# biaslab/GaussianProcessNode

Hardware: AMD Instinct MI355X
Metric: VMP iterations/sec (sparse-GP node sweep, kin40k-shaped synthetic) (higher is better)
Workload: dtype f64

## Files before the change

### gaussianprocessnode_amd/csrc/sgp_api.hip

```cpp
#include "../../include/sgp_hip.h"
#include "sgp_kernels.hip.h"
#include "point_scratch.h"

#include <algorithm>
#include <atomic>
#include <chrono>
#include <cmath>
#include <cstdio>
#include <cstdlib>
#include <dlfcn.h>
#include <cstring>
#include <limits>
#include <mutex>
#include <string>
#include <type_traits>
#include <vector>

using namespace sgp;

namespace {

thread_local std::string g_create_error;
std::atomic<int> g_live_handles{0};

// ... 20 lines not shown
    std::lock_guard<std::mutex> lock(g_registry_mutex);
    auto& r = registry();
    auto it = std::find(r.begin(), r.end(), h);
    if (it == r.end()) return false;
    r.erase(it);
    return true;
}

}

enum { WORD_JOIN = 0,
       WORD_DONE = 1,
       WORD_GATE = 2,
       WORD_GRAD = 3,
       WORD_ASM0 = 4,
       WORD_GROUP0 = 8,
       WORD_COUNT = 8 + LAM_MAX_GROUPS };
constexpr int RESERVED_CUS_PER_SE = 2;

struct StatGroup {
    int c0, c1;
    int row_lo, nrows;
    int ntiles;
    SyrkGeom geom;
    int form_step;
    bool early;
    bool masked;
    size_t slab_off;
};

struct SweepPlan {
    hipStream_t stream = nullptr;
    bool overlapped = false;
    bool pack = false;
    bool events = false;
    bool join_word = false;
    bool kuu_interleaved = false;
    bool resident = false;
};

struct StatsRecord {
    double sigma2 = 0.0, jitter = 0.0, inv_ell[MAXD] = {0};
    int32_t family = SGP_KERNEL_SE;
    uint64_t data_gen = ~0ull;
    double w0 = 1.0;
    bool qv = false;
    bool reusable = false;
    bool checked = false;
    bool targets = false;
    bool exact_psi = false;
};
// ... 295 lines not shown
                               tv_xi, tv_t, mu_acc, uv_part, none);
        }
        ++j;
    }
};
static void launch_potrf(double* A, int ld, int Tn, int* info, int n_valid, double* scratch, hipStream_t s,
                         double* Winv = nullptr, const LamForm* form = nullptr, double* Sacc = nullptr,
                         const double* tv_xi = nullptr, double* tv_t = nullptr, const hipEvent_t* step_wait = nullptr) {
    PotrfSeq q(A, ld, Tn, info, n_valid, scratch, s, Winv, form, Sacc, tv_xi, tv_t, step_wait);
    while (!q.done()) q.next();
}

static void launch_ata(const double* W, double* C, int ld, int Tn, hipStream_t s, int rev = 0, double* mu = nullptr,
                       double* R = nullptr, const double* Psi2 = nullptr, const double* Kinv = nullptr,
                       double* trace_part = nullptr, const UvArgs* uv = nullptr, const double* Sacc = nullptr) {
    const int extra = uv ? Tn * Tn : 0;
    hipLaunchKernelGGL(k_gemm32, dim3(Tn * (Tn + 1) / 2 * 4 + extra), dim3(256), 0, s, W, W, C, ld, Tn, 0, 0, rev, mu, R, Psi2,
                       Kinv, trace_part, uv ? *uv : UvArgs{}, Sacc);
}
static void launch_gemm(const double* A, const double* B, double* C, int ld, int Tn, hipStream_t s) {
    hipLaunchKernelGGL(k_gemm32, dim3(Tn * Tn * 4), dim3(256), 0, s, A, B, C, ld, Tn, 3, 0, 0, (double*)nullptr, (double*)nullptr,
                       (const double*)nullptr, (const double*)nullptr, (double*)nullptr, UvArgs{}, (const double*)nullptr);
}


extern "C" int sgp_abi_version(void) { return SGP_ABI_VERSION; }

extern "C" const char* sgp_last_error(const sgp_handle* h) { return h ? h->err.c_str() : g_create_error.c_str(); }

template <typename T>
static hipError_t dalloc(T** p, size_t count) {
// ... 598 lines not shown
                           int64_t* stamps = nullptr, const long long* wait_word = nullptr, long long wait_need = 0,
                           const long long* gate_word = nullptr, long long gate_need = 0, int* sync_status = nullptr) {
    hipLaunchKernelGGL(k_prep_xu, dim3((h->Mp + 255) / 256), dim3(256), 0, s, h->dXu, Xus, src, dP, info_reset, h->M, h->Mp, h->D, stamps,
                       stamps ? (int)SGP_T_COUNT : 0, stamps ? (int)SGP_T_SWEEP : 0, wait_word, wait_need, gate_word, gate_need,
                       h->spin_limit, sync_status);
}
static void mirror_current_params(sgp_handle* h, hipStream_t s) { launch_prep_xu(h, s, h->dXusK, h->hParams, h->dParamsK); }

static void kuu_gram(sgp_handle* h, hipStream_t s, bool gate) {
    by_family(h->family, [&](auto F) {
        constexpr int FAM = decltype(F)::value;
        if (gate) hipLaunchKernelGGL(k_gram_uu_lds<FAM>, dim3(h->T, h->T), dim3(256), 0, s, h->dXusK, h->dKuu, h->dParamsK, h->M, h->Mp, h->D);
        else hipLaunchKernelGGL(k_gram_uu<FAM>, dim3(h->T, h->T), dim3(256), 0, s, h->dXusK, h->dKuu, h->dParamsK, h->M, h->Mp, h->D);
    });
}
static void kuu_tail(sgp_handle* h, hipStream_t s, bool join_word) {
    launch_ata(h->dWk, h->dKinv, h->Mp, h->T, s, 0, nullptr, nullptr, nullptr, nullptr, nullptr, nullptr, h->dSaccK);
    if (join_word) hipLaunchKernelGGL(k_join_set, dim3(1), dim3(64), 0, s, h->dJoin + WORD_JOIN, h->join_epoch);
}
static void enqueue_kuu_head(sgp_handle* h, hipStream_t s) {
    const bool words = s == h->side;
    const bool gate = words && h->gate_side;
    launch_prep_xu(h, s, h->dXusK, h->params_src, h->dParamsK, h->dInfo + 0, nullptr, words ? h->dJoin + WORD_DONE : nullptr,
                   h->done_epoch, gate ? h->dJoin + WORD_GATE : nullptr, h->gate_epoch, h->dInfo + 3);
    kuu_gram(h, s, gate);
}
static void enqueue_kuu(sgp_handle* h, hipStream_t s, bool join_word) {
    enqueue_kuu_head(h, s);
    launch_potrf(h->dKuu, h->Mp, h->T, h->dInfo + 0, h->M, h->dScratch, s, h->dWk, nullptr, h->dSaccK);
    kuu_tail(h, s, join_word);
}

static void launch_gram_uf(const sgp_handle* h, hipStream_t s, const double* Xus, const double* X, const double* Yw, double* Kuf,
                           double* bpart, const Params* P, int64_t N, int d_out, int64_t* stamps, int64_t* sweep_begin) {
    const dim3 grid((unsigned)((N + TB - 1) / TB), h->T);
    by_family(h->family, [&](auto F) {
        auto launch = [&](auto DCAP) {
            hipLaunchKernelGGL(HIP_KERNEL_NAME(k_gram_uf<decltype(DCAP)::value, decltype(F)::value>), grid, dim3(256), 0, s, Xus, X, Yw,
                               Kuf, bpart, P, h->M, h->Mp, h->D, N, d_out, stamps, sweep_begin);
        };
        if (h->D <= 8) launch(std::integral_constant<int, 8>{});
        else launch(std::integral_constant<int, MAXD>{});
    });
}
static void launch_gram(sgp_handle* h, hipStream_t s, bool stamped) {
// ... 51 lines not shown
            hipLaunchKernelGGL(k_join_set, dim3(1), dim3(64), 0, s, h->dJoin + WORD_GROUP0 + g, h->stat_epoch);
    }
    return 0;
}

static void enqueue_finish1(sgp_handle* h, hipStream_t s, const SweepPlan& p) {
    const int M = h->M, Mp = h->Mp, Q = h->Q, Qp = h->Qp, TQ = h->TQ;
    LamForm form;
    memset(&form, 0, sizeof form);
    form.stats = h->dStats; form.Lambda0 = h->dLambda0; form.xi0 = h->dXi0; form.xi = h->dXi; form.P = h->dParams;
    form.M = M; form.Mp = Mp; form.d_out = h->dout; form.Q = Q; form.prior_form = h->prior_form;
    form.stamps = h->dStamps + STAMP_STRIDE * SGP_T_FINISH1;
    form.spin_limit = h->spin_limit;
    form.sync_status = h->dInfo + 3;
    form.trace_chain = 1;
    hipEvent_t step_wait[LAM_MAX_COLS] = {nullptr};
    bool any_wait = false;
    if (p.overlapped) {
        form.col_words = h->dJoin + WORD_GROUP0;
        form.col_need = h->stat_epoch;
        for (int g = 0; g < h->ngroups; ++g) {
            for (int c = h->grp[g].c0; c < h->grp[g].c1; ++c) {
                form.form_step[c] = (unsigned char)(h->grp[g].form_step | (h->grp[g].early ? LAM_FORM_EARLY : 0));
                form.col_group[c] = (h->grp[g].masked && !p.pack && !p.resident) ? (unsigned char)g : (unsigned char)0xff;
            }
            if (h->grp[g].masked && p.pack && !p.resident) { step_wait[h->grp[g].form_step - (h->grp[g].early ? 1 : 0)] = h->evGroup[g]; any_wait = true; }
        }
    }
    double* uvt0 = h->dUvWork + 2 * (size_t)Qp;
    PotrfSeq lam(h->dLam, Qp, TQ, h->dInfo + 1, Qp, h->dScratch + POTRF_SCRATCH, s, h->dWl, &form, h->dTmp, h->dXi, uvt0,
                 any_wait ? step_wait : nullptr);
    lam.mu_acc = h->dUvWork;
    lam.uv_part = uvt0 + (size_t)TQ * Qp;
    if (p.kuu_interleaved) {
        PotrfSeq kuu(h->dKuu, h->Mp, h->T, h->dInfo + 0, h->M, h->dScratch, h->side, h->dWk, nullptr, h->dSaccK);
        while (!lam.done() || !kuu.done()) {
            if (!lam.done()) lam.next();
            if (!kuu.done()) kuu.next();
        }
        kuu_tail(h, h->side, p.join_word);
    } else {
        while (!lam.done()) lam.next();
    }
}

static double* mirror_for(const sgp_handle* h) {
    return (h->hMirror && !h->env_no_zero_copy && !h->training) ? h->hMirror : nullptr;
}

static void launch_traces(sgp_handle* h, hipStream_t s, const double* Rv = nullptr) {
    hipLaunchKernelGGL(k_trace_kinv, dim3(TRACE_BLOCKS), dim3(256), 0, s, h->dStats, h->dKinv, h->dTrace, h->M, h->Mp);
    hipLaunchKernelGGL(k_trace_R, dim3(TRACE_BLOCKS), dim3(256), 0, s, h->dStats, Rv ? Rv : h->dR, h->dTrace + TRACE_BLOCKS, h->M, h->Mp, h->dout,
                       h->Qp, (int64_t*)nullptr);
}

static void enqueue_finish2(sgp_handle* h, hipStream_t s, bool join_word) {
    const int M = h->M, Mp = h->Mp, Q = h->Q, Qp = h->Qp, TQ = h->TQ;
    double* uvt = h->dUvWork + 2 * (size_t)Qp;
    double* uvpart = uvt + (size_t)TQ * Qp;
    const int nata = TQ * (TQ + 1) / 2 * 4;
    double* traceR = h->dTrace + TRACE_BLOCKS;
    const double* partK = h->dTrace;
    int nK = TRACE_BLOCKS, nR = TRACE_BLOCKS;
    UvArgs uv;
    uv.Wp = h->dWl; uv.t = uvt; uv.muacc = h->dUvWork; uv.partial = uvpart; uv.LR = h->dUvT;
    uv.stamps = h->dStamps + STAMP_STRIDE * SGP_T_FINISH1;
    uv.join = join_word ? h->dJoin + WORD_JOIN : nullptr;
    uv.join_need = h->join_epoch;
    uv.spin_limit = h->spin_limit;
    uv.sync_status = h->dInfo + 3;
    if (h->dout == 1) {
        launch_ata(h->dWl, h->dSigma, Qp, TQ, s, 1, h->dMu, h->dR, h->dStats, h->dKinv, traceR, &uv, h->dTmp);
        partK = traceR + nata;
        nK = nR = nata;
    } else {
        launch_ata(h->dWl, h->dSigma, Qp, TQ, s, 1, h->dMu, h->dR, nullptr, nullptr, nullptr, &uv, h->dTmp);
        launch_traces(h, s);
    }
    hipLaunchKernelGGL(k_scalars, dim3(1), dim3(256), 0, s, h->dStats, partK, nK, (const double*)traceR, nR, h->dMu, h->dKuu,
                       h->dLam, h->dInfo, h->dParams, h->dOut, h->dWishart, M, Mp, h->dout, Q, Qp, Qp - Q,
                       h->dStamps + STAMP_STRIDE * SGP_T_FINISH2, h->dStamps, h->dStampTotals,
                       h->dJoin + WORD_DONE, h->done_epoch,
                       (const double*)(h->dScratch + POTRF_LOGDET), h->T, (const double*)(h->dScratch + POTRF_SCRATCH + POTRF_LOGDET), TQ,
                       mirror_for(h));
}

static int set_device_checked(int device) {
    int ndev = 0;
    if (hipGetDeviceCount(&ndev) != hipSuccess || ndev == 0) return fail(nullptr, SGP_ERR_NODEVICE, "no HIP device visible");
    if (device < 0 || device >= ndev) return fail(nullptr, SGP_ERR_ARG, "bad device ordinal");
    if (hipSetDevice(device) != hipSuccess) return fail(nullptr, SGP_ERR_HIP, "hipSetDevice failed");
    return 0;
}

namespace {
struct EventPair {
    hipEvent_t a = nullptr, b = nullptr;
    ~EventPair() { if (a) hipEventDestroy(a); if (b) hipEventDestroy(b); }
    hipError_t create() { hipError_t e = hipEventCreate(&a); return e != hipSuccess ? e : hipEventCreate(&b); }
// ... 39 lines not shown
    SweepPlan p;
    p.stream = stream ? static_cast<hipStream_t>(stream) : h->own;
    p.events = h->allreduce != nullptr || p.stream != h->own;
    p.overlapped = whole && h->overlap && !stream && (h->n > 0 || h->allreduce) && !h->training;
    p.pack = whole && h->allreduce != nullptr;
    return p;
}

static int sweep_local_impl(sgp_handle* h, void* stream, bool whole, bool need_data = true) {
    int rc = check_ready(h, need_data);
    if (rc) return rc;
    HIPCHK(h, hipSetDevice(h->cfg.device));
    SweepPlan p = sweep_plan(h, stream, whole);
    if (int brc = sweep_begin(h)) return brc;
    if (p.events) HIPCHK(h, hipStreamWaitEvent(h->side, h->evDone, 0));
    {
        const int grid = h->TQ * (h->TQ + 1) / 2 * 4 + h->TQ * h->TQ;
        p.join_word = h->dout == 1 && !p.events && grid <= h->num_cus - 40 && g_live_handles.load() <= 1;
        ++h->join_epoch;
    }
    ++h->gate_epoch;
    if (p.overlapped) ++h->stat_epoch;
    const bool stats_first = h->gate_side && h->n > 0 && !h->allreduce;
    p.kuu_interleaved = whole && h->env_interleave && stats_first && !p.events;
    h->plan = p;
    auto enqueue_stats = [&]() -> int {
        if (p.overlapped) {
            if (int orc = enqueue_stats_overlapped(h, p)) return orc;
        } else
            enqueue_local(h, p.stream, p.pack);
        HIPCHK(h, hipGetLastError());
        return 0;
    };
    if (stats_first)
        if (int src = enqueue_stats()) return src;
    if (p.kuu_interleaved)
        enqueue_kuu_head(h, h->side);
    else
        enqueue_kuu(h, h->side, p.join_word);
    HIPCHK(h, hipGetLastError());
    if (!p.kuu_interleaved) HIPCHK(h, hipEventRecord(h->evSide, h->side));
    if (!stats_first)
        if (int src = enqueue_stats()) return src;
    stats_formed(h);
    return 0;
}

extern "C" int sgp_sweep_local(sgp_handle* h, void* stream) {
    const int rc = sweep_local_impl(h, stream, false);
    if (h) stats_drop(h, STATS_REUSE);
    return rc;
}

extern "C" int sgp_sweep_finish(sgp_handle* h, void* stream) {
    if (!h) return SGP_ERR_ARG;
    if (!h->swept_local) return fail(h, SGP_ERR_ARG, "sgp_sweep_finish: call sgp_sweep_local first");
    HIPCHK(h, hipSetDevice(h->cfg.device));
    hipStream_t s = stream ? static_cast<hipStream_t>(stream) : h->own;
    const SweepPlan p = h->plan;
    h->plan.overlapped = h->plan.kuu_interleaved = false;
    h->in_flight = true;
    enqueue_finish1(h, s, p);
    HIPCHK(h, hipGetLastError());
    if (p.kuu_interleaved) HIPCHK(h, hipEventRecord(h->evSide, h->side));
    if (!p.join_word) HIPCHK(h, hipStreamWaitEvent(s, h->evSide, 0));
    return sweep_close(h, s, p, p.join_word);
}

static int exchange_stats(sgp_handle* h, hipStream_t s, int tile0, int ntile, bool with_tail) {
    const int tail = (int)(h->Mp * h->dout + SGP_S_COUNT + h->dout * h->dout);
    const int64_t count = (int64_t)ntile * TB * TB + (with_tail ? tail : 0);
    if (with_tail && tile0 + ntile != h->ntiles) return fail(h, SGP_ERR_ARG, "internal: the tail of the exchange buffer follows its last tile");
    if (h->allreduce(h->allreduce_ctx, h->dPack + (size_t)tile0 * TB * TB, count, s))
        return fail(h, SGP_ERR_HIP, "the all-reduce hook failed (statistics)");
    hipLaunchKernelGGL(k_unpack_stats, dim3(ntile + 1), dim3(256), 0, s, (const double*)h->dPack, h->dStats, h->Mp, h->T,
                       with_tail ? tail : 0, tile0, ntile);
    HIPCHK(h, hipGetLastError());
    return 0;
}
// ... 186 lines not shown

static bool mirror_fresh(const sgp_handle* h) {
    return h->hMirror && h->mirror_epoch >= 0 && h->mirror_epoch == h->done_epoch && !h->sync_reported &&
           h->hMirror[SGP_R_COUNT + 1] == (double)h->mirror_epoch;
}

static int check_sync_status(sgp_handle* h) {
    if (mirror_fresh(h) && h->hMirror[SGP_R_COUNT] == 0.0) return 0;
    int bits = 0;
    HIPCHK(h, hipMemcpy(&bits, h->dInfo + 3, sizeof(int), hipMemcpyDeviceToHost));
    if (bits == 0) return 0;
    h->sync_reported = true;
    std::string msg = "a bounded device-word wait gave up (stream hand-off not honoured; results refused):";
    if (bits & SYNC_LATE_DONE) msg += " [done word: the next sweep's first kernels started before the previous sweep had finished]";
    if (bits & SYNC_LATE_GRAD_START) msg += " [done word: the K_uu half of the theta gradient started before the sweep had finished]";
    if (bits & SYNC_LATE_KINV) msg += " [join word: the Sigma launch did not get K_uu^-1 from the K_uu chain]";
    if (bits & SYNC_LATE_GRAD_JOIN) msg += " [gradient word: the K_uu half of the theta gradient did not arrive]";
    if (bits & SYNC_LATE_COLUMN) msg += " [statistics words: a Lambda-chain step did not get its tile columns / the masked stream did not get K_uf]";
    h->err = msg;
    return SGP_ERR_HIP;
}

static int sync_checked(sgp_handle* h) {
    if (int rc = sync_all(h)) return rc;
    return check_sync_status(h);
}

static int last_sweep_status(sgp_handle* h, const char* name_kuu, const char* name_lambda) {
    if (int src = check_sync_status(h)) return src;
    int info[2];
    HIPCHK(h, hipMemcpy(info, h->dInfo, sizeof info, hipMemcpyDeviceToHost));
    return factor_status(h, info[0], name_kuu, info[1], name_lambda, true);
}
// ... 904 lines not shown
        if (int rrc = theta_Rv(h, s, &R)) return rrc;
    const int64_t nprep = std::max<int64_t>(h->n, Mp);
    hipLaunchKernelGGL(k_theta_multi_prep, dim3((unsigned)((nprep + 255) / 256)), dim3(256), 0, s, (const double*)h->dYw,
                       (const double*)h->dMu, w.W, cw, mup, h->n, M, Mp, dout);
    hipLaunchKernelGGL(k_form_G_multi, dim3(Mp), dim3(256), 0, s, R, Qp, (const double*)h->dKinv, (const double*)h->dStats,
                       w.W, w.trace, h->dGradM, part, M, Mp, dout);
    hipLaunchKernelGGL(k_theta_value_multi, dim3(1), dim3(256), 0, s, (const double*)part, (const double*)h->dStats,
                       (const double*)mup, (const Params*)h->dParams, w.W, w.trace, h->dGrad + GRAD_SLOTS, Mp, dout);
    HIPCHK(h, hipGetLastError());
    return 0;
}

static int enqueue_restats(sgp_handle* h, hipStream_t s) {
    stats_drop(h, STATS_REUSE | STATS_QV);
    h->swept_local = true;
    enqueue_kuu(h, s, false);
    enqueue_local(h, s, h->allreduce != nullptr);
    if (h->allreduce)
        if (int xrc = exchange_stats(h, s)) return xrc;
    force_prep_main(h);
    return 0;
}

static int theta_objective_multi(sgp_handle* h, hipStream_t s, bool fresh, double* value, double* grad) {
    if (fresh) {
        double out[SGP_R_COUNT];
        HIPCHK(h, hipMemcpy(out, h->dOut, sizeof out, hipMemcpyDeviceToHost));
        if (int frc = factor_status(h, (int)out[SGP_R_INFO_KUU], "K_uu")) return frc;
    } else {
        if (int erc = enqueue_restats(h, s)) return erc;
        HIPCHK(h, hipStreamSynchronize(s));
// ... 9 lines not shown
    HIPCHK(h, hipGetLastError());
    double res[GRAD_SLOTS + 1];
    HIPCHK(h, hipMemcpy(res, h->dGrad, sizeof res, hipMemcpyDeviceToHost));
    *value = res[GRAD_SLOTS];
    if (grad)
        for (int i = 0; i <= h->n_ell; ++i) grad[i] = res[i];
    return 0;
}

static void enqueue_theta_uni_sums(sgp_handle* h, hipStream_t s, const double* Rv) {
    const int M = h->M, Mp = h->Mp, Q = h->Q, Qp = h->Qp;
    launch_traces(h, s, Rv);
    hipLaunchKernelGGL(k_scalars, dim3(1), dim3(256), 0, s, h->dStats, (const double*)h->dTrace, (int)TRACE_BLOCKS,
                       (const double*)(h->dTrace + TRACE_BLOCKS), (int)TRACE_BLOCKS, h->dMu, h->dKuu, h->dLam, h->dInfo, h->dParams,
                       h->dOut2, h->dWishart, M, Mp, h->dout, Q, Qp, Qp - Q, (int64_t*)nullptr, (int64_t*)nullptr,
                       (int64_t*)nullptr, (long long*)nullptr, 0LL, (const double*)nullptr, 0, (const double*)nullptr, 0, (double*)nullptr);
}

static int theta_objective_eval(sgp_handle* h, hipStream_t s, double* value, const double** Rv_out) {
    if (int erc = enqueue_restats(h, s)) return erc;
    const int Mp = h->Mp;
    const double* Rv = h->dR;
    if (int rrc = theta_Rv(h, s, &Rv)) return rrc;
    *Rv_out = Rv;
    enqueue_theta_uni_sums(h, s, Rv);
    HIPCHK(h, hipStreamSynchronize(s));
    HIPCHK(h, hipGetLastError());
    double out[SGP_R_COUNT], sc[SGP_S_COUNT];
    HIPCHK(h, hipMemcpy(out, h->dOut2, sizeof out, hipMemcpyDeviceToHost));
    HIPCHK(h, hipMemcpy(sc, h->dStats + (size_t)Mp * Mp + (size_t)Mp * h->dout, sizeof sc, hipMemcpyDeviceToHost));
    if (int frc = factor_status(h, (int)out[SGP_R_INFO_KUU], "K_uu")) return frc;
// ... 841 lines not shown
```

### gaussianprocessnode_amd/csrc/sgp_kernels.hip.h

```cpp
#pragma once
#include <hip/hip_runtime.h>
#include <stdint.h>
#include <utility>

namespace sgp {

constexpr int TB = 64;
constexpr int PS = 80;
constexpr int KB = 16;
constexpr int MAXD = 32;
constexpr int MAXO = 4;
constexpr int LT = TB + 1;

typedef double d4 __attribute__((ext_vector_type(4)));

struct Params {
    double sigma2;
    double jitter;
    double E_logw;
    double n_override;
    double inv_ell[MAXD];
    double W[MAXO * MAXO];
    double prior_iso;
    double pad[7];
// ... 1213 lines not shown
constexpr int LAM_FORM_EARLY = 0x80;
struct LamForm {
    const double* stats;
    const double* Lambda0;
    const double* xi0;
    double* xi;
    const Params* P;
    int M, Mp, d_out, Q, prior_form;
    int64_t* stamps;
    const long long* col_words;
    long long col_need;
    unsigned char form_step[LAM_MAX_COLS], col_group[LAM_MAX_COLS];
    int spin_limit;
    int* sync_status;
    int trace_chain;
};
__device__ __forceinline__ double load_agent(const double* p) {
    return __hip_atomic_load((const __attribute__((address_space(1))) double*)p, __ATOMIC_RELAXED, __HIP_MEMORY_SCOPE_AGENT);
}
template <bool DENSE, bool MULTI, bool BYPASS = false>
__device__ __forceinline__ double lambda_entry(const LamForm& f, int gi, int gj, int Qp, double prior_iso, double w00) {
    const bool inside = gi < f.Q && gj < f.Q;
    const int si = inside ? gi : 0, sj = inside ? gj : 0;
    int a = 0, i = si, b = 0, j = sj;
    if constexpr (MULTI) { a = si / f.M; i = si % f.M; b = sj / f.M; j = sj % f.M; }
    double psi;
    if constexpr (BYPASS) psi = load_agent(f.stats + (size_t)j * f.Mp + i); else psi = f.stats[(size_t)j * f.Mp + i];
    const double diag = (gi == gj) ? 1.0 : 0.0;
    double prior, w;
    if constexpr (DENSE) prior = f.Lambda0[(size_t)sj * Qp + si]; else prior = diag * prior_iso;
// ... 496 lines not shown
    };
    TileRegs rX, rS, rD;
    if (lam && j == 0) stamp_enter(form.stamps);
    STEP_TRACE(0);
    if (panel) {
        long long* tw_words = reinterpret_cast<long long*>(scratch + 3 * TB * TB);
        if (!xgroup) {
            if (a != 0 || diag_inv) __builtin_amdgcn_s_setprio(3);
            tile_fetch(rS, do_form, load_old, A, form, ld, j0, j0, bypass);
            if (j > 0) {
                tile_g2r(rD, Dn_in, TB, 0, 0);
#pragma unroll
                for (int u = 0; u < 16; ++u) rS.v[u] -= rD.v[u];
            }
            if (xi_duty) form_xi(form, ld, tid, bypass);
            if (a == 0 && tid == 0) tw_words[(j + 1) & 1] = 0;
            tile_r2s(S, rS);
            STEP_TRACE(1);
            __syncthreads();
            STEP_TRACE(2);
            if (a == 0 && j > 0 && !diag_inv) move_prev();
            const bool has_solve = (a != 0) || diag_inv;
            const int ntwf = 1 + potrf_twins(Tn, j);
            static_assert(10 <= 2 * 2 * (1 + POTRF_TWINS), "two tiles of X X^T per wave must cover the ten lower tiles");
            int fcount = 0, fR[2], fC[2];
            d4 fg[2];
#pragma unroll
            for (int q = 0; q < 2; ++q) {
                fg[q] = (d4){0.0, 0.0, 0.0, 0.0};
                fR[q] = fC[q] = 0;
                const int t = tw + ntwf * ((wave - 1) + 2 * q);
// ... 159 lines not shown
#pragma unroll
    for (int u = 0; u < 32; ++u) {
        const double2 w = src[u];
        v[63 - 2 * u] = w.x;
        v[62 - 2 * u] = w.y;
    }
}

struct UvArgs {
    const double* Wp;
    const double* t;
    const double* muacc;
    const double* partial;
    double* LR;
    int64_t* stamps;
    const long long* join;
    long long join_need;
    int spin_limit;
    int* sync_status;
};
__global__ void k_join_wait(const long long* w, long long need, int spin_limit, int* sync_status, int bit, int trace_slot) {
    TraceScope trace(trace_slot);
    if (threadIdx.x == 0 && blockIdx.x == 0) spin_until(w, need, spin_limit, sync_status, bit);
}
__global__ void k_join_set(long long* w, long long v) {
    if (threadIdx.x == 0 && blockIdx.x == 0)
        __hip_atomic_store((__attribute__((address_space(1))) long long*)w, v, __ATOMIC_RELAXED, __HIP_MEMORY_SCOPE_AGENT);
}
__device__ __forceinline__ void uv_cols_role(const UvArgs& u, int Qp, int kb, int jb) {
    const int lane = threadIdx.x, j = 64 * jb + lane;
    double* out = u.LR + (size_t)(64 * kb) * Qp + j;
    if (kb > jb) {
#pragma unroll 16
        for (int kk = 0; kk < 64; ++kk) out[(size_t)kk * Qp] = 0.0;
        stamp_exit(u.stamps);
        return;
    }
    double v[64];
    load_v_column(v, u.Wp, Qp, kb, j);
    double T = 0.0;
// ... 35 lines not shown
        T = fma(lane_value(pl, kk), v[kk], T);
    }
    stamp_exit(u.stamps);
}

__global__ void __launch_bounds__(256) k_gemm32(const double* __restrict__ A, const double* __restrict__ B, double* __restrict__ C,
                                                int ld, int Tn, int mode, int s, int rev, double* __restrict__ mu,
                                                double* __restrict__ R, const double* __restrict__ Psi2,
                                                const double* __restrict__ Kinv, double* __restrict__ trace_part, UvArgs uv,
                                                const double* __restrict__ Sacc) {
    __shared__ double As[64 * PS32];
    __shared__ double Bs[64 * PS32];
    __shared__ double tred[4];
    __shared__ double mup[4 * 64], mus[64];
    TraceScope trace(mode == 0 ? (mu ? 5 : 6) : 255);
    if (mode == 0 && uv.Wp) {
        const int ngemm = Tn * (Tn + 1) / 2 * 4;
        if ((int)blockIdx.x >= ngemm) {
            if (threadIdx.x >= 64) return;
            const int e = blockIdx.x - ngemm;
            uv_cols_role(uv, ld, e % Tn, e / Tn);
            return;
        }
    }
    const int tid = threadIdx.x, lane = tid & 63, wave = tid >> 6, wr = wave >> 1, wc = wave & 1;
    const int quad = blockIdx.x & 3, qi = quad >> 1, qj = quad & 1;
    int I, J, kbeg, kend;
    if (mode == 0) {
        tile_from_index(blockIdx.x >> 2, I, J);
        kbeg = Sacc ? max(I, Tn - 2) : I;
        kend = Tn;
    } else {
        const int t = blockIdx.x >> 2;
        I = t / Tn; J = t % Tn; kbeg = 0; kend = Tn;
    }
    const int r0 = I * TB + qi * 32, c0 = J * TB + qj * 32;
    d4 acc = (d4){0.0, 0.0, 0.0, 0.0};
    const int li = lane & 15, lk = lane >> 4;
    if (mode == 0 && Sacc && I < Tn - 2) {
#pragma unroll
        for (int r = 0; r < 4; ++r) acc[r] = Sacc[(size_t)(c0 + wc * 16 + li) * ld + r0 + wr * 16 + lk + 4 * r];
    }
    const int oc = tid >> 3, o4 = (tid & 7) * 4;
    const int gcA = rev ? ld - 1 - (c0 + oc) : c0 + oc, grA = rev ? ld - 1 - (r0 + o4 + 3) : r0 + o4;
    const int gcB = rev ? ld - 1 - (r0 + oc) : r0 + oc, grB = rev ? ld - 1 - (c0 + o4 + 3) : c0 + o4;
    const size_t offA = (size_t)gcA * ld + grA, offB = (size_t)gcB * ld + grB;
    double2 p0 = make_double2(0.0, 0.0), p1 = p0, q0 = p0, q1 = p0;
    double muA[5] = {0.0, 0.0, 0.0, 0.0, 0.0}, muB[5] = {0.0, 0.0, 0.0, 0.0, 0.0};
    const int me = tid & 63;
    double mt[16], mbase = 0.0;
    bool kinv_late = false;
    if (mode == 0 && mu) {
#pragma unroll
        for (int u = 0; u < 16; ++u) mt[u] = uv.t[(Tn - 1) * TB + 16 * wave + u];
        if (wave == 0 && ((me < 32) ? I : J) < Tn - 1) mbase = uv.muacc[(me < 32) ? r0 + me : c0 + me - 32];
        if (Psi2) {
            p0 = *reinterpret_cast<const double2*>(Psi2 + offA); p1 = *reinterpret_cast<const double2*>(Psi2 + offA + 2);
            kinv_late = uv.join && !join_ready(uv.join, uv.join_need);
            if (!kinv_late) { q0 = *reinterpret_cast<const double2*>(Kinv + offA); q1 = *reinterpret_cast<const double2*>(Kinv + offA + 2); }
        }
    }
    for (int k = kbeg; k < kend; ++k) {
        __syncthreads();
        if (mode == 0) load_panel32_t(As, A, ld, k * TB, r0, tid);
        else load_panel32_n(As, A, ld, r0, k * TB, tid);
        load_panel32_t(Bs, B, ld, k * TB, c0, tid);
        __syncthreads();
        const double* ap = As + lk * PS32 + wr * 16 + li;
        const double* bp = Bs + lk * PS32 + wc * 16 + li;
#pragma unroll
        for (int k4 = 0; k4 < 16; ++k4) acc = __builtin_amdgcn_mfma_f64_16x16x4f64(ap[k4 * 4 * PS32], bp[k4 * 4 * PS32], acc, 0, 0, 0);
    }
    if (mode == 0 && mu) {
        const double* pan = ((me < 32) ? As + me : Bs + me - 32) + 16 * wave * PS32;
        double sdot = 0.0;
// ... 26 lines not shown
    }
    {
        double v[4];
#pragma unroll
        for (int e = 0; e < 4; ++e) v[e] = Qd[oc * 33 + o4 + (rev ? 3 - e : e)];
        *reinterpret_cast<double2*>(C + offA) = make_double2(v[0], v[1]);
        *reinterpret_cast<double2*>(C + offA + 2) = make_double2(v[2], v[3]);
        if (mu) {
            double rv[4];
#pragma unroll
            for (int e = 0; e < 4; ++e) rv[e] = fma(muA[e], muA[4], v[e]);
            *reinterpret_cast<double2*>(R + offA) = make_double2(rv[0], rv[1]);
            *reinterpret_cast<double2*>(R + offA + 2) = make_double2(rv[2], rv[3]);
            if (Psi2) {
                tsum = fma(rv[0], p0.x, fma(rv[1], p0.y, fma(rv[2], p1.x, rv[3] * p1.y)));
                if (kinv_late) {
                    if (spin_until(uv.join, uv.join_need, uv.spin_limit, uv.sync_status, SYNC_LATE_KINV)) {
                        const __attribute__((address_space(1))) double* kq = (const __attribute__((address_space(1))) double*)(Kinv + offA);
                        q0.x = __hip_atomic_load(kq + 0, __ATOMIC_RELAXED, __HIP_MEMORY_SCOPE_AGENT);
                        q0.y = __hip_atomic_load(kq + 1, __ATOMIC_RELAXED, __HIP_MEMORY_SCOPE_AGENT);
                        q1.x = __hip_atomic_load(kq + 2, __ATOMIC_RELAXED, __HIP_MEMORY_SCOPE_AGENT);
                        q1.y = __hip_atomic_load(kq + 3, __ATOMIC_RELAXED, __HIP_MEMORY_SCOPE_AGENT);
                    } else
                        q0.x = __builtin_nan("");
                }
                tsumK = fma(q0.x, p0.x, fma(q0.y, p0.y, fma(q1.x, p1.x, q1.y * p1.y)));
            }
        }
    }
    {
        double v[4];
#pragma unroll
        for (int e = 0; e < 4; ++e) v[e] = Qd[(o4 + (rev ? 3 - e : e)) * 33 + oc];
        *reinterpret_cast<double2*>(C + offB) = make_double2(v[0], v[1]);
        *reinterpret_cast<double2*>(C + offB + 2) = make_double2(v[2], v[3]);
        if (mu) {
            double rv[4];
#pragma unroll
            for (int e = 0; e < 4; ++e) rv[e] = fma(muB[e], muB[4], v[e]);
            *reinterpret_cast<double2*>(R + offB) = make_double2(rv[0], rv[1]);
            *reinterpret_cast<double2*>(R + offB + 2) = make_double2(rv[2], rv[3]);
        }
    }
    if (trace_part) {
        if (I != J) { tsum *= 2.0; tsumK *= 2.0; }
        tsum = block_sum(tsum, tred);
        tsumK = block_sum(tsumK, tred);
        if (tid == 0) {
            trace_part[blockIdx.x] = tsum;
            trace_part[Tn * (Tn + 1) / 2 * 4 + blockIdx.x] = tsumK;
        }
    }
}

__global__ void __launch_bounds__(256) k_symv(const double* __restrict__ S, const double* __restrict__ x,
                                              double* __restrict__ y, int n, int ld) {
    const int row = blockIdx.x * 4 + (threadIdx.x >> 6), lane = threadIdx.x & 63;
    if (row >= n) return;
    double s = 0.0;
    for (int j = lane; j < n; j += 64) s = fma(S[(size_t)row * ld + j], x[j], s);
    for (int o = 32; o > 0; o >>= 1) s += __shfl_xor(s, o);
    if (lane == 0) y[row] = s;
}

constexpr int CU_MAXQ = 4096;
// ... 29 lines not shown
                    t2 = fma(R[(size_t)(b * M + j) * Qp + a * M + i], Psi2[(size_t)j * Mp + i], t2);
            t2 = block_sum(t2, red);
            if (tid == 0) partial[(size_t)blockIdx.x * d_out * d_out + a + b * d_out] = t2;
        }
}

__global__ void __launch_bounds__(256) k_scalars(const double* __restrict__ stats, const double* __restrict__ partK, int nK,
                                                 const double* __restrict__ partR, int nR,
                                                 const double* __restrict__ mu, const double* __restrict__ Lkuu,
                                                 const double* __restrict__ Llam, const int* __restrict__ info,
                                                 const Params* __restrict__ P, double* __restrict__ out,
                                                 double* __restrict__ wishart, int M, int Mp, int d_out, int Q, int Qp,
                                                 int lam_off, int64_t* stamps, int64_t* all_stamps,
                                                 int64_t* totals, long long* done_word, long long done_value,
                                                 const double* __restrict__ ldK, int nldK, const double* __restrict__ ldL, int nldL,
                                                 double* __restrict__ mirror) {
    __shared__ double red[4];
    __shared__ double redn[4 * 5];
    __shared__ double tr[TRACE_SLOTS];
    TraceScope trace(7);
    stamp_enter(stamps);
    const double* B = stats + (size_t)Mp * Mp;
    const double* sc = B + (size_t)Mp * d_out;
    const int tid = threadIdx.x;
    if (d_out == 1) {
        StampFold fold = {0, 0, 0};
        if (all_stamps && tid >= 192) fold = stamp_fold_load(all_stamps, totals, tid - 192);
        const double c_syy = sc[0], c_skk = sc[1], c_n = sc[2], c_w = P->W[0], c_sigma2 = P->sigma2, c_elogw = P->E_logw;
        const int c_i0 = info[0], c_i1 = info[1], c_i2 = info[2], c_i3 = mirror ? info[3] : 0;
        double v[5] = {0.0, 0.0, 0.0, 0.0, 0.0};
        for (int b = tid; b < nK; b += 256) v[0] += partK[b];
        for (int b = tid; b < nR; b += 256) v[1] += partR[b];
        for (int e = tid; e < M; e += 256) {
            if (!ldK) v[2] += log(Lkuu[(size_t)e * Mp + e]);
            v[4] = fma(B[e], mu[e], v[4]);
        }
        if (ldK) for (int e = tid; e < nldK; e += 256) v[2] += ldK[e];
        if (ldL) for (int e = tid; e < nldL; e += 256) v[3] += ldL[e];
        else for (int e = tid; e < Q; e += 256) v[3] += log(Llam[(size_t)(e + lam_off) * Qp + e + lam_off]);
#pragma unroll
        for (int i = 0; i < 5; ++i)
            for (int o = 32; o > 0; o >>= 1) v[i] += __shfl_xor(v[i], o);
        if ((tid & 63) == 0)
#pragma unroll
            for (int i = 0; i < 5; ++i) redn[(tid >> 6) * 5 + i] = v[i];
        __syncthreads();
        if (tid == 0) {
            double t[5];
#pragma unroll
            for (int i = 0; i < 5; ++i) t[i] = (redn[i] + redn[5 + i]) + (redn[10 + i] + redn[15 + i]);
            const double LOG2PI = 1.8378770664093454835606594728112;
            const double n = c_n, w = c_w;
            const double sum_I1 = c_sigma2 * c_skk - t[0];
            const double sum_I2 = c_syy - 2.0 * t[4] + t[1];
// ... 2336 lines not shown
```

Before: 4835.

## Move K_uu trace term into Kinv launch and defer join to scalars kernel

The K_uu^-1 tail launch now also computes the trace(Kinv·Psi2) partials itself. It spin-waits on a new stats word that the Lambda-chain's first step publishes, plus any masked group words. The Sigma launch no longer waits on the join word for Kinv; only the closing scalars kernel spins on it to collect the traces and log-determinant. When the plan is not interleaved, the tail launch is deferred to the finish phase. The join-word path is also no longer gated by a CU-count budget, which takes the K_uu chain off the Sigma launch's critical path. The cost is extra device-word spinning and a risk of co-residency deadlock on the spin waits.

Result: no change. 4840, median of 6 (+0.1%).

```diff
diff --git a/gaussianprocessnode_amd/csrc/sgp_api.hip b/gaussianprocessnode_amd/csrc/sgp_api.hip
--- a/gaussianprocessnode_amd/csrc/sgp_api.hip
+++ b/gaussianprocessnode_amd/csrc/sgp_api.hip
@@ -58,6 +58,7 @@
        WORD_GATE = 2,
        WORD_GRAD = 3,
        WORD_ASM0 = 4,
+       WORD_STATS0 = 5,
        WORD_GROUP0 = 8,
        WORD_COUNT = 8 + LAM_MAX_GROUPS };
 constexpr int RESERVED_CUS_PER_SE = 2;
@@ -79,6 +80,7 @@
     bool pack = false;
     bool events = false;
     bool join_word = false;
+    bool kuu_tail_pending = false;
     bool kuu_interleaved = false;
     bool resident = false;
 };
@@ -404,7 +406,7 @@
 static void launch_ata(const double* W, double* C, int ld, int Tn, hipStream_t s, int rev = 0, double* mu = nullptr,
                        double* R = nullptr, const double* Psi2 = nullptr, const double* Kinv = nullptr,
                        double* trace_part = nullptr, const UvArgs* uv = nullptr, const double* Sacc = nullptr) {
-    const int extra = uv ? Tn * Tn : 0;
+    const int extra = (uv && uv->Wp) ? Tn * Tn : 0;
     hipLaunchKernelGGL(k_gemm32, dim3(Tn * (Tn + 1) / 2 * 4 + extra), dim3(256), 0, s, W, W, C, ld, Tn, 0, 0, rev, mu, R, Psi2,
                        Kinv, trace_part, uv ? *uv : UvArgs{}, Sacc);
 }
@@ -1033,9 +1035,23 @@
         else hipLaunchKernelGGL(k_gram_uu<FAM>, dim3(h->T, h->T), dim3(256), 0, s, h->dXusK, h->dKuu, h->dParamsK, h->M, h->Mp, h->D);
     });
 }
-static void kuu_tail(sgp_handle* h, hipStream_t s, bool join_word) {
-    launch_ata(h->dWk, h->dKinv, h->Mp, h->T, s, 0, nullptr, nullptr, nullptr, nullptr, nullptr, nullptr, h->dSaccK);
-    if (join_word) hipLaunchKernelGGL(k_join_set, dim3(1), dim3(64), 0, s, h->dJoin + WORD_JOIN, h->join_epoch);
+static double* kshares_of(const sgp_handle* h) { return h->dTrace + TRACE_BLOCKS + h->TQ * (h->TQ + 1) / 2 * 4; }
+static void kuu_tail(sgp_handle* h, hipStream_t s, const SweepPlan& p) {
+    if (p.join_word) {
+        UvArgs uv{};
+        uv.stat_word = h->dJoin + WORD_STATS0;
+        uv.stat_need = h->join_epoch;
+        uv.group_words = h->dJoin + WORD_GROUP0;
+        uv.group_need = h->stat_epoch;
+        if (p.overlapped && !p.pack)
+            for (int g = 0; g < h->ngroups; ++g)
+                if (h->grp[g].masked) uv.group_mask |= 1u << g;
+        uv.spin_limit = h->spin_limit;
+        uv.sync_status = h->dInfo + 3;
+        launch_ata(h->dWk, h->dKinv, h->Mp, h->T, s, 0, nullptr, nullptr, h->dStats, nullptr, kshares_of(h), &uv, h->dSaccK);
+        hipLaunchKernelGGL(k_join_set, dim3(1), dim3(64), 0, s, h->dJoin + WORD_JOIN, h->join_epoch, 11);
+    } else
+        launch_ata(h->dWk, h->dKinv, h->Mp, h->T, s, 0, nullptr, nullptr, nullptr, nullptr, nullptr, nullptr, h->dSaccK);
 }
 static void enqueue_kuu_head(sgp_handle* h, hipStream_t s) {
     const bool words = s == h->side;
@@ -1044,10 +1060,10 @@
                    h->done_epoch, gate ? h->dJoin + WORD_GATE : nullptr, h->gate_epoch, h->dInfo + 3);
     kuu_gram(h, s, gate);
 }
-static void enqueue_kuu(sgp_handle* h, hipStream_t s, bool join_word) {
+static void enqueue_kuu(sgp_handle* h, hipStream_t s, const SweepPlan& p, bool tail) {
     enqueue_kuu_head(h, s);
     launch_potrf(h->dKuu, h->Mp, h->T, h->dInfo + 0, h->M, h->dScratch, s, h->dWk, nullptr, h->dSaccK);
-    kuu_tail(h, s, join_word);
+    if (tail) kuu_tail(h, s, p);
 }
 
 static void launch_gram_uf(const sgp_handle* h, hipStream_t s, const double* Xus, const double* X, const double* Yw, double* Kuf,
@@ -1129,6 +1145,7 @@
     form.spin_limit = h->spin_limit;
     form.sync_status = h->dInfo + 3;
     form.trace_chain = 1;
+    if (p.join_word) { form.stats0_word = h->dJoin + WORD_STATS0; form.stats0_value = h->join_epoch; }
     hipEvent_t step_wait[LAM_MAX_COLS] = {nullptr};
     bool any_wait = false;
     if (p.overlapped) {
@@ -1153,7 +1170,7 @@
             if (!lam.done()) lam.next();
             if (!kuu.done()) kuu.next();
         }
-        kuu_tail(h, h->side, p.join_word);
+        kuu_tail(h, h->side, p);
     } else {
         while (!lam.done()) lam.next();
     }
@@ -1180,12 +1197,13 @@
     UvArgs uv;
     uv.Wp = h->dWl; uv.t = uvt; uv.muacc = h->dUvWork; uv.partial = uvpart; uv.LR = h->dUvT;
     uv.stamps = h->dStamps + STAMP_STRIDE * SGP_T_FINISH1;
-    uv.join = join_word ? h->dJoin + WORD_JOIN : nullptr;
-    uv.join_need = h->join_epoch;
+    uv.stat_word = uv.group_words = nullptr;
+    uv.stat_need = uv.group_need = 0;
+    uv.group_mask = 0;
     uv.spin_limit = h->spin_limit;
     uv.sync_status = h->dInfo + 3;
     if (h->dout == 1) {
-        launch_ata(h->dWl, h->dSigma, Qp, TQ, s, 1, h->dMu, h->dR, h->dStats, h->dKinv, traceR, &uv, h->dTmp);
+        launch_ata(h->dWl, h->dSigma, Qp, TQ, s, 1, h->dMu, h->dR, h->dStats, join_word ? nullptr : h->dKinv, traceR, &uv, h->dTmp);
         partK = traceR + nata;
         nK = nR = nata;
     } else {
@@ -1197,7 +1215,8 @@
                        h->dStamps + STAMP_STRIDE * SGP_T_FINISH2, h->dStamps, h->dStampTotals,
                        h->dJoin + WORD_DONE, h->done_epoch,
                        (const double*)(h->dScratch + POTRF_LOGDET), h->T, (const double*)(h->dScratch + POTRF_SCRATCH + POTRF_LOGDET), TQ,
-                       mirror_for(h));
+                       mirror_for(h), join_word ? (const long long*)(h->dJoin + WORD_JOIN) : (const long long*)nullptr, h->join_epoch,
+                       h->spin_limit, h->dInfo + 3);
 }
 
 static int set_device_checked(int device) {
@@ -1267,15 +1286,13 @@
     SweepPlan p = sweep_plan(h, stream, whole);
     if (int brc = sweep_begin(h)) return brc;
     if (p.events) HIPCHK(h, hipStreamWaitEvent(h->side, h->evDone, 0));
-    {
-        const int grid = h->TQ * (h->TQ + 1) / 2 * 4 + h->TQ * h->TQ;
-        p.join_word = h->dout == 1 && !p.events && grid <= h->num_cus - 40 && g_live_handles.load() <= 1;
-        ++h->join_epoch;
-    }
+    p.join_word = h->dout == 1 && !p.events && g_live_handles.load() <= 1;
+    ++h->join_epoch;
     ++h->gate_epoch;
     if (p.overlapped) ++h->stat_epoch;
     const bool stats_first = h->gate_side && h->n > 0 && !h->allreduce;
     p.kuu_interleaved = whole && h->env_interleave && stats_first && !p.events;
+    p.kuu_tail_pending = p.join_word && !p.kuu_interleaved;
     h->plan = p;
     auto enqueue_stats = [&]() -> int {
         if (p.overlapped) {
@@ -1290,7 +1307,7 @@
     if (p.kuu_interleaved)
         enqueue_kuu_head(h, h->side);
     else
-        enqueue_kuu(h, h->side, p.join_word);
+        enqueue_kuu(h, h->side, p, !p.kuu_tail_pending);
     HIPCHK(h, hipGetLastError());
     if (!p.kuu_interleaved) HIPCHK(h, hipEventRecord(h->evSide, h->side));
     if (!stats_first)
@@ -1311,11 +1328,12 @@
     HIPCHK(h, hipSetDevice(h->cfg.device));
     hipStream_t s = stream ? static_cast<hipStream_t>(stream) : h->own;
     const SweepPlan p = h->plan;
-    h->plan.overlapped = h->plan.kuu_interleaved = false;
+    h->plan.overlapped = h->plan.kuu_interleaved = h->plan.kuu_tail_pending = h->plan.join_word = false;
     h->in_flight = true;
+    if (p.kuu_tail_pending) kuu_tail(h, h->side, p);
     enqueue_finish1(h, s, p);
     HIPCHK(h, hipGetLastError());
-    if (p.kuu_interleaved) HIPCHK(h, hipEventRecord(h->evSide, h->side));
+    if (p.kuu_interleaved || p.kuu_tail_pending) HIPCHK(h, hipEventRecord(h->evSide, h->side));
     if (!p.join_word) HIPCHK(h, hipStreamWaitEvent(s, h->evSide, 0));
     return sweep_close(h, s, p, p.join_word);
 }
@@ -1532,9 +1550,9 @@
     std::string msg = "a bounded device-word wait gave up (stream hand-off not honoured; results refused):";
     if (bits & SYNC_LATE_DONE) msg += " [done word: the next sweep's first kernels started before the previous sweep had finished]";
     if (bits & SYNC_LATE_GRAD_START) msg += " [done word: the K_uu half of the theta gradient started before the sweep had finished]";
-    if (bits & SYNC_LATE_KINV) msg += " [join word: the Sigma launch did not get K_uu^-1 from the K_uu chain]";
+    if (bits & SYNC_LATE_KINV) msg += " [join word: the sweep's closing kernel did not get the K_uu chain's traces and log-determinant]";
     if (bits & SYNC_LATE_GRAD_JOIN) msg += " [gradient word: the K_uu half of the theta gradient did not arrive]";
-    if (bits & SYNC_LATE_COLUMN) msg += " [statistics words: a Lambda-chain step did not get its tile columns / the masked stream did not get K_uf]";
+    if (bits & SYNC_LATE_COLUMN) msg += " [statistics words: a Lambda-chain step or the K_uu^-1 launch did not get its statistics / the masked stream did not get K_uf]";
     h->err = msg;
     return SGP_ERR_HIP;
 }
@@ -2469,7 +2487,7 @@
 static int enqueue_restats(sgp_handle* h, hipStream_t s) {
     stats_drop(h, STATS_REUSE | STATS_QV);
     h->swept_local = true;
-    enqueue_kuu(h, s, false);
+    enqueue_kuu(h, s, SweepPlan{}, true);
     enqueue_local(h, s, h->allreduce != nullptr);
     if (h->allreduce)
         if (int xrc = exchange_stats(h, s)) return xrc;
@@ -2509,7 +2527,8 @@
     hipLaunchKernelGGL(k_scalars, dim3(1), dim3(256), 0, s, h->dStats, (const double*)h->dTrace, (int)TRACE_BLOCKS,
                        (const double*)(h->dTrace + TRACE_BLOCKS), (int)TRACE_BLOCKS, h->dMu, h->dKuu, h->dLam, h->dInfo, h->dParams,
                        h->dOut2, h->dWishart, M, Mp, h->dout, Q, Qp, Qp - Q, (int64_t*)nullptr, (int64_t*)nullptr,
-                       (int64_t*)nullptr, (long long*)nullptr, 0LL, (const double*)nullptr, 0, (const double*)nullptr, 0, (double*)nullptr);
+                       (int64_t*)nullptr, (long long*)nullptr, 0LL, (const double*)nullptr, 0, (const double*)nullptr, 0, (double*)nullptr,
+                       (const long long*)nullptr, 0LL, 0, (int*)nullptr);
 }
 
 static int theta_objective_eval(sgp_handle* h, hipStream_t s, double* value, const double** Rv_out) {
diff --git a/gaussianprocessnode_amd/csrc/sgp_kernels.hip.h b/gaussianprocessnode_amd/csrc/sgp_kernels.hip.h
--- a/gaussianprocessnode_amd/csrc/sgp_kernels.hip.h
+++ b/gaussianprocessnode_amd/csrc/sgp_kernels.hip.h
@@ -1251,6 +1251,8 @@
     int spin_limit;
     int* sync_status;
     int trace_chain;
+    long long* stats0_word;
+    long long stats0_value;
 };
 __device__ __forceinline__ double load_agent(const double* p) {
     return __hip_atomic_load((const __attribute__((address_space(1))) double*)p, __ATOMIC_RELAXED, __HIP_MEMORY_SCOPE_AGENT);
@@ -1777,7 +1779,11 @@
                 for (int u = 0; u < 16; ++u) rS.v[u] -= rD.v[u];
             }
             if (xi_duty) form_xi(form, ld, tid, bypass);
-            if (a == 0 && tid == 0) tw_words[(j + 1) & 1] = 0;
+            if (a == 0 && tid == 0) {
+                tw_words[(j + 1) & 1] = 0;
+                if (j == 0 && form.stats0_word)
+                    __hip_atomic_store((__attribute__((address_space(1))) long long*)form.stats0_word, form.stats0_value, __ATOMIC_RELAXED, __HIP_MEMORY_SCOPE_AGENT);
+            }
             tile_r2s(S, rS);
             STEP_TRACE(1);
             __syncthreads();
@@ -1967,8 +1973,10 @@
     const double* partial;
     double* LR;
     int64_t* stamps;
-    const long long* join;
-    long long join_need;
+    const long long* stat_word;
+    const long long* group_words;
+    long long stat_need, group_need;
+    unsigned group_mask;
     int spin_limit;
     int* sync_status;
 };
@@ -1976,7 +1984,8 @@
     TraceScope trace(trace_slot);
     if (threadIdx.x == 0 && blockIdx.x == 0) spin_until(w, need, spin_limit, sync_status, bit);
 }
-__global__ void k_join_set(long long* w, long long v) {
+__global__ void k_join_set(long long* w, long long v, int trace_slot = 255) {
+    TraceScope trace(trace_slot);
     if (threadIdx.x == 0 && blockIdx.x == 0)
         __hip_atomic_store((__attribute__((address_space(1))) long long*)w, v, __ATOMIC_RELAXED, __HIP_MEMORY_SCOPE_AGENT);
 }
@@ -2042,10 +2051,10 @@
     __shared__ double tred[4];
     __shared__ double mup[4 * 64], mus[64];
     TraceScope trace(mode == 0 ? (mu ? 5 : 6) : 255);
-    if (mode == 0 && uv.Wp) {
+    if (mode == 0) {
         const int ngemm = Tn * (Tn + 1) / 2 * 4;
         if ((int)blockIdx.x >= ngemm) {
-            if (threadIdx.x >= 64) return;
+            if (!uv.Wp || threadIdx.x >= 64) return;
             const int e = blockIdx.x - ngemm;
             uv_cols_role(uv, ld, e % Tn, e / Tn);
             return;
@@ -2073,20 +2082,31 @@
     const int gcA = rev ? ld - 1 - (c0 + oc) : c0 + oc, grA = rev ? ld - 1 - (r0 + o4 + 3) : r0 + o4;
     const int gcB = rev ? ld - 1 - (r0 + oc) : r0 + oc, grB = rev ? ld - 1 - (c0 + o4 + 3) : c0 + o4;
     const size_t offA = (size_t)gcA * ld + grA, offB = (size_t)gcB * ld + grB;
-    double2 p0 = make_double2(0.0, 0.0), p1 = p0, q0 = p0, q1 = p0;
+    double2 p0 = make_double2(0.0, 0.0), p1 = p0, q0 = p0, q1 = p0, pk0 = p0, pk1 = p0;
     double muA[5] = {0.0, 0.0, 0.0, 0.0, 0.0}, muB[5] = {0.0, 0.0, 0.0, 0.0, 0.0};
     const int me = tid & 63;
     double mt[16], mbase = 0.0;
-    bool kinv_late = false;
     if (mode == 0 && mu) {
 #pragma unroll
         for (int u = 0; u < 16; ++u) mt[u] = uv.t[(Tn - 1) * TB + 16 * wave + u];
         if (wave == 0 && ((me < 32) ? I : J) < Tn - 1) mbase = uv.muacc[(me < 32) ? r0 + me : c0 + me - 32];
         if (Psi2) {
             p0 = *reinterpret_cast<const double2*>(Psi2 + offA); p1 = *reinterpret_cast<const double2*>(Psi2 + offA + 2);
-            kinv_late = uv.join && !join_ready(uv.join, uv.join_need);
-            if (!kinv_late) { q0 = *reinterpret_cast<const double2*>(Kinv + offA); q1 = *reinterpret_cast<const double2*>(Kinv + offA + 2); }
-        }
+            if (Kinv) {
+                const size_t offK = (size_t)(c0 + oc) * ld + r0 + o4;
+                q0 = *reinterpret_cast<const double2*>(Kinv + offK); q1 = *reinterpret_cast<const double2*>(Kinv + offK + 2);
+                pk0 = *reinterpret_cast<const double2*>(Psi2 + offK); pk1 = *reinterpret_cast<const double2*>(Psi2 + offK + 2);
+            }
+        }
+    }
+    const bool kshare = mode == 0 && !mu && Psi2 && trace_part;
+    bool stats_late = false;
+    if (kshare) {
+        if (uv.stat_word) {
+            stats_late = !join_ready(uv.stat_word, uv.stat_need);
+            for (unsigned m = uv.group_mask; m; m &= m - 1) stats_late |= !join_ready(uv.group_words + (__ffs(m) - 1), uv.group_need);
+        }
+        if (!stats_late) { p0 = *reinterpret_cast<const double2*>(Psi2 + offA); p1 = *reinterpret_cast<const double2*>(Psi2 + offA + 2); }
     }
     for (int k = kbeg; k < kend; ++k) {
         __syncthreads();
@@ -2143,18 +2163,21 @@
             *reinterpret_cast<double2*>(R + offA + 2) = make_double2(rv[2], rv[3]);
             if (Psi2) {
                 tsum = fma(rv[0], p0.x, fma(rv[1], p0.y, fma(rv[2], p1.x, rv[3] * p1.y)));
-                if (kinv_late) {
-                    if (spin_until(uv.join, uv.join_need, uv.spin_limit, uv.sync_status, SYNC_LATE_KINV)) {
-                        const __attribute__((address_space(1))) double* kq = (const __attribute__((address_space(1))) double*)(Kinv + offA);
-                        q0.x = __hip_atomic_load(kq + 0, __ATOMIC_RELAXED, __HIP_MEMORY_SCOPE_AGENT);
-                        q0.y = __hip_atomic_load(kq + 1, __ATOMIC_RELAXED, __HIP_MEMORY_SCOPE_AGENT);
-                        q1.x = __hip_atomic_load(kq + 2, __ATOMIC_RELAXED, __HIP_MEMORY_SCOPE_AGENT);
-                        q1.y = __hip_atomic_load(kq + 3, __ATOMIC_RELAXED, __HIP_MEMORY_SCOPE_AGENT);
-                    } else
-                        q0.x = __builtin_nan("");
-                }
-                tsumK = fma(q0.x, p0.x, fma(q0.y, p0.y, fma(q1.x, p1.x, q1.y * p1.y)));
-            }
+                if (Kinv) tsumK = fma(q0.x, pk0.x, fma(q0.y, pk0.y, fma(q1.x, pk1.x, q1.y * pk1.y)));
+            }
+        }
+        if (kshare) {
+            if (stats_late) {
+                bool ok = spin_until(uv.stat_word, uv.stat_need, uv.spin_limit, uv.sync_status, SYNC_LATE_COLUMN);
+                for (unsigned m = uv.group_mask; m; m &= m - 1)
+                    ok = spin_until(uv.group_words + (__ffs(m) - 1), uv.group_need, uv.spin_limit, uv.sync_status, SYNC_LATE_COLUMN) && ok;
+                if (ok) {
+                    p0.x = load_agent(Psi2 + offA + 0); p0.y = load_agent(Psi2 + offA + 1);
+                    p1.x = load_agent(Psi2 + offA + 2); p1.y = load_agent(Psi2 + offA + 3);
+                } else
+                    p0.x = __builtin_nan("");
+            }
+            tsumK = fma(v[0], p0.x, fma(v[1], p0.y, fma(v[2], p1.x, v[3] * p1.y)));
         }
     }
     {
@@ -2173,11 +2196,16 @@
     }
     if (trace_part) {
         if (I != J) { tsum *= 2.0; tsumK *= 2.0; }
+        if (kshare) {
+            tsumK = block_sum(tsumK, tred);
+            if (tid == 0) trace_part[blockIdx.x] = tsumK;
+            return;
+        }
         tsum = block_sum(tsum, tred);
-        tsumK = block_sum(tsumK, tred);
+        if (Kinv) tsumK = block_sum(tsumK, tred);
         if (tid == 0) {
             trace_part[blockIdx.x] = tsum;
-            trace_part[Tn * (Tn + 1) / 2 * 4 + blockIdx.x] = tsumK;
+            if (Kinv) trace_part[Tn * (Tn + 1) / 2 * 4 + blockIdx.x] = tsumK;
         }
     }
 }
@@ -2237,7 +2265,8 @@
                                                  int lam_off, int64_t* stamps, int64_t* all_stamps,
                                                  int64_t* totals, long long* done_word, long long done_value,
                                                  const double* __restrict__ ldK, int nldK, const double* __restrict__ ldL, int nldL,
-                                                 double* __restrict__ mirror) {
+                                                 double* __restrict__ mirror, const long long* join, long long join_need,
+                                                 int spin_limit, int* sync_status) {
     __shared__ double red[4];
     __shared__ double redn[4 * 5];
     __shared__ double tr[TRACE_SLOTS];
@@ -2250,17 +2279,35 @@
         StampFold fold = {0, 0, 0};
         if (all_stamps && tid >= 192) fold = stamp_fold_load(all_stamps, totals, tid - 192);
         const double c_syy = sc[0], c_skk = sc[1], c_n = sc[2], c_w = P->W[0], c_sigma2 = P->sigma2, c_elogw = P->E_logw;
-        const int c_i0 = info[0], c_i1 = info[1], c_i2 = info[2], c_i3 = mirror ? info[3] : 0;
+        const int c_i1 = info[1], c_i2 = info[2];
         double v[5] = {0.0, 0.0, 0.0, 0.0, 0.0};
-        for (int b = tid; b < nK; b += 256) v[0] += partK[b];
         for (int b = tid; b < nR; b += 256) v[1] += partR[b];
-        for (int e = tid; e < M; e += 256) {
-            if (!ldK) v[2] += log(Lkuu[(size_t)e * Mp + e]);
-            v[4] = fma(B[e], mu[e], v[4]);
-        }
-        if (ldK) for (int e = tid; e < nldK; e += 256) v[2] += ldK[e];
+        for (int e = tid; e < M; e += 256) v[4] = fma(B[e], mu[e], v[4]);
         if (ldL) for (int e = tid; e < nldL; e += 256) v[3] += ldL[e];
         else for (int e = tid; e < Q; e += 256) v[3] += log(Llam[(size_t)(e + lam_off) * Qp + e + lam_off]);
+        bool late = false, arrived = true;
+        if (join && !join_ready(join, join_need)) {
+            late = true;
+            arrived = spin_until(join, join_need, spin_limit, sync_status, SYNC_LATE_KINV);
+        }
+        int c_i0, c_i3 = 0;
+        if (!late) {
+            c_i0 = info[0];
+            if (mirror) c_i3 = info[3];
+            for (int b = tid; b < nK; b += 256) v[0] += partK[b];
+            if (ldK) for (int e = tid; e < nldK; e += 256) v[2] += ldK[e];
+            else for (int e = tid; e < M; e += 256) v[2] += log(Lkuu[(size_t)e * Mp + e]);
+        } else {
+            const __attribute__((address_space(1))) int* ginfo = (const __attribute__((address_space(1))) int*)info;
+            c_i0 = __hip_atomic_load(ginfo + 0, __ATOMIC_RELAXED, __HIP_MEMORY_SCOPE_AGENT);
+            if (mirror) c_i3 = __hip_atomic_load(ginfo + 3, __ATOMIC_RELAXED, __HIP_MEMORY_SCOPE_AGENT) | (arrived ? 0 : (int)SYNC_LATE_KINV);
+            if (arrived) {
+                for (int b = tid; b < nK; b += 256) v[0] += load_agent(partK + b);
+                if (ldK) for (int e = tid; e < nldK; e += 256) v[2] += load_agent(ldK + e);
+                else for (int e = tid; e < M; e += 256) v[2] += log(load_agent(Lkuu + (size_t)e * Mp + e));
+            } else
+                v[0] = v[2] = __builtin_nan("");
+        }
 #pragma unroll
         for (int i = 0; i < 5; ++i)
             for (int o = 32; o > 0; o >>= 1) v[i] += __shfl_xor(v[i], o);
```
